# RuntimeRacer/vall-e

Measured on AMD Instinct MI355X. Metric: AR codec-tokens/sec/GPU + NAR 7-stage p50 latency, d=1024 L=12 10s utterance, higher is better.
Workload: dtype bf16

## Files before the change

vall-e_amd/csrc/ar_granules.hpp:

```cpp
#pragma once
#include "ar_kernels.hpp"

namespace vx {

constexpr int FQ_G = 16;
constexpr int FQ_QKV = 192;
constexpr int FQ_PART = 66;
constexpr int FQ_SPIN_MAX = 1 << 18;

typedef unsigned long long fq_gran;

#ifdef VX_STAMPS
}
extern __device__ unsigned long long* g_fq_stamps;
namespace vx {
#endif

__device__ __forceinline__ void gran_store(fq_gran* p, float v, unsigned tag) {
  const fq_gran g = ((fq_gran)tag << 32) | (fq_gran)__float_as_uint(v);
  asm volatile("global_store_dwordx2 %0, %1, off sc1" ::"v"(p), "v"(g) : "memory");
}
__device__ __forceinline__ void gran_load(fq_gran& v, const fq_gran* p) {
  asm volatile("global_load_dwordx2 %0, %1, off sc1" : "=v"(v) : "v"(p) : "memory");
}
// ... 27 lines not shown
```

vall-e_amd/csrc/ar_tp.hpp:

```cpp
#pragma once
#include <type_traits>
#include "ar_granules.hpp"

namespace vx {

#ifdef VX_STAMPS
#define TP_STAMP(which, i)                                                                                            \
  do {                                                                                                                \
    unsigned long long* fq_r_ = g_fq_stamps;                                                                          \
    if (fq_r_ != nullptr && threadIdx.x == 0)                                                                         \
      fq_r_[(((size_t)(which) * 16 + a.layer) * 256 + blockIdx.x) * 16 + (i)] = __builtin_amdgcn_s_memrealtime();      \
  } while (0)
#else
#define TP_STAMP(which, i) do { } while (0)
#endif

constexpr int TP_D = 1024, TP_H = 16, TP_FF = 4096, TP_X = 8, TP_WG = 32;
constexpr int TP_HID = TP_FF / TP_X;
constexpr int TP_ACH = TP_D / TP_X;

struct TpAccArgs {
  long long* add;
  long long* zero;
  const float* bias;
// ... 78 lines not shown
  float s1 = wave_sum_dpp((v.x + v.y) + (v.z + v.w));
  if (lane == 0) red[wave] = s1;
  __syncthreads();
  const float mean = ((red[0] + red[1]) + (red[2] + red[3])) * (1.0f / TP_D);
  const float d0 = v.x - mean, d1 = v.y - mean, d2 = v.z - mean, d3 = v.w - mean;
  float s2 = wave_sum_dpp((d0 * d0 + d1 * d1) + (d2 * d2 + d3 * d3));
  if (lane == 0) red[4 + wave] = s2;
  __syncthreads();
  const float rstd = 1.0f / sqrtf(((red[4] + red[5]) + (red[6] + red[7])) * (1.0f / TP_D) + LN_EPS);
  *reinterpret_cast<float4*>(xs + 4 * tid) =
      make_float4(d0 * rstd * r.g.x + r.be.x, d1 * rstd * r.g.y + r.be.y, d2 * rstd * r.g.z + r.be.z, d3 * rstd * r.g.w + r.be.w);
  __syncthreads();
}

template <bool FIRST>
__device__ __forceinline__ void tp_acc_tail(const TpAccArgs& a, float partial, int xcd, int i, int tid, unsigned long long carry_ll,
                                            float carry_f, float bo) {
  if ((tid & 7) == 0) {
    long long add = tp_fix(partial);
    if (xcd == 0) add += tp_fix(bo) + (FIRST ? tp_fix(carry_f) : (long long)carry_ll);
    atomicAdd(reinterpret_cast<unsigned long long*>(a.add) + 32 * i + (tid >> 3), (unsigned long long)add);
  }
  if (blockIdx.x == 1) {
    *reinterpret_cast<uint4*>(a.zero + 4 * tid) = make_uint4(0u, 0u, 0u, 0u);
    *reinterpret_cast<uint4*>(a.zero + 4 * tid + 2) = make_uint4(0u, 0u, 0u, 0u);
  }
}

template <int KCH, int VEC>
__device__ __forceinline__ void tp_row_read(const float* xs, int lane, float (&xr)[KCH][VEC]) {
#pragma unroll
  for (int c = 0; c < KCH; ++c)
#pragma unroll
    for (int i = 0; i < VEC; i += 4) {
      const float4 t = *reinterpret_cast<const float4*>(xs + (c * 64 + lane) * VEC + i);
      xr[c][i] = t.x; xr[c][i + 1] = t.y; xr[c][i + 2] = t.z; xr[c][i + 3] = t.w;
// ... 1 lines not shown
}
template <typename WT, int KCH>
__device__ __forceinline__ float tp_dot(const uint4 (&w)[KCH], const float (&xr)[KCH][Vec16<WT>::N]) {
  constexpr int VEC = Vec16<WT>::N;
  float s = 0.f;
#pragma unroll
  for (int c = 0; c < KCH; ++c) {
    float wf[VEC];
    unpack<WT>(w[c], wf);
#pragma unroll
    for (int i = 0; i < VEC; ++i) s = fmaf(wf[i], xr[c][i], s);
  }
  return s;
}

template <typename WT, bool FIRST>
__global__ __launch_bounds__(256) void tp_attn_kernel(const void* __restrict__ Wqkv_, const float* __restrict__ x_f32,
                                                      const long long* __restrict__ racc, const float* __restrict__ gbb,
                                                      const ArState* __restrict__ st, const unsigned* __restrict__ epoch,
                                                      const void* __restrict__ Wo_, const TpAttnArgs a) {
  constexpr int VEC = Vec16<WT>::N;
  constexpr int KCH = TP_D / (64 * VEC);
  constexpr int HD = 64;
  constexpr int LPK = HD / VEC, KPW = 64 / LPK, KPB = 4 * KPW, UNR = 4;
  constexpr int NGRP = 4 * KPW;
  constexpr int OCH = TP_ACH / (8 * VEC);
  __shared__ __attribute__((aligned(16))) float xs[TP_D];
  __shared__ float red[8];
  __shared__ __attribute__((aligned(16))) float s_qkv[FQ_QKV];
  __shared__ __attribute__((aligned(16))) float sm_o[NGRP][HD + 4];
  __shared__ float sm_m[4], sm_l[4];
  __shared__ float s_wo[4][HD];
  __shared__ float s_part[2 * FQ_G * FQ_PART];
  __shared__ float s_fac[2 * FQ_G];
  __shared__ __attribute__((aligned(16))) float s_att[TP_ACH];
  const int tid = threadIdx.x, lane = tid & 63, wave = tid >> 6;
  const int x = blockIdx.x & (TP_X - 1), i = blockIdx.x >> 3;
  const int hl = i >> 4, j = i & 15, h = 2 * x + hl;
  const int cih = 4 * j + wave, ch = h * HD + cih;
  const int st_row = st->row, st_done = st->done;
  const unsigned tag = *epoch;
  const WT* __restrict__ W = reinterpret_cast<const WT*>(Wqkv_);

  TpRowLoads rl;
  tp_row_issue<FIRST>(rl, x_f32, racc, gbb, tid);
  TP_STAMP(0, 0);
  vx_u32x4 w[3][KCH];
#pragma unroll
  for (int r = 0; r < 3; ++r)
#pragma unroll
    for (int c = 0; c < KCH; ++c) tp_ld16w(w[r][c], W + (size_t)(r * TP_D + ch) * TP_D + (c * 64 + lane) * VEC);
  float e_bias;
  {
    const float* bp = a.qkv_bias;
    asm volatile("" : "+s"(bp));
    tp_ld4f(e_bias, bp + min(lane, 2) * TP_D + ch);
  }
  unsigned long long carry_ll = 0ull;
  float carry_f = 0.f, bo;
  if (FIRST) tp_ld4f(carry_f, x_f32 + 32 * i + (tid >> 3));
  else asm volatile("global_load_dwordx2 %0, %1, off" : "=v"(carry_ll) : "v"(racc + 32 * i + (tid >> 3)) : "memory");
  tp_ld4f(bo, a.acc.bias + 32 * i + (tid >> 3));
  const int n_old = st_row;
  const int chunk = (n_old + FQ_G - 1) / FQ_G;
  const int j0 = j * chunk, j1 = min(n_old, j0 + chunk);
  const int sub = lane % LPK, grp = lane / LPK;
  vx_u32x4 wo[OCH];
  vx_u32x4 kr[UNR], vr[UNR];
  const WT* kb;
  const WT* vb;
  auto tp_stage2 = [&]() {
    const uint4* wb = reinterpret_cast<const uint4*>(Wo_) + (size_t)(x * TP_WG + i) * OCH * 256;
#pragma unroll
    for (int m = 0; m < OCH; ++m) tp_ld16w(wo[m], wb + m * 256 + tid);
    const void* kcp = a.kcache;
    const void* vcp = a.vcache;
    int ctxm = a.ctx_max;
    asm volatile("" : "+s"(kcp), "+s"(vcp), "+s"(ctxm));
    kb = reinterpret_cast<const WT*>(kcp) + (size_t)h * ctxm * HD + sub * VEC;
    vb = reinterpret_cast<const WT*>(vcp) + (size_t)h * ctxm * HD + sub * VEC;
#pragma unroll
    for (int u = 0; u < UNR; ++u) {
      const int jk = min(j0 + u * KPB + wave * KPW + grp, max(j1, 1) - 1);
      tp_ld16(kr[u], kb + (size_t)jk * HD);
      tp_ld16(vr[u], vb + (size_t)jk * HD);
    }
  };
  tp_stage2();
  auto load_pass = [&](int base) {
#pragma unroll
    for (int u = 0; u < UNR; ++u) {
      const int jk = min(base + u * KPB + wave * KPW + grp, max(j1, 1) - 1);
      const uint4 k4 = ld16(kb + (size_t)jk * HD), v4 = ld16(vb + (size_t)jk * HD);
      kr[u] = vx_u32x4{k4.x, k4.y, k4.z, k4.w};
      vr[u] = vx_u32x4{v4.x, v4.y, v4.z, v4.w};
    }
  };
  constexpr int N_KV = 2 * UNR, N_WO = OCH, N_W = 3 * KCH;

  tp_row_wait<FIRST, N_W + 3 + N_WO + N_KV>(rl);
  TP_STAMP(0, 7);
  tp_row_norm<FIRST>(rl, xs, red, tid);
  TP_STAMP(0, 1);
  {
    float xr[KCH][VEC];
    tp_row_read<KCH, VEC>(xs, lane, xr);
    float acc[3];
#pragma unroll
    for (int r = 0; r < 3; ++r) {
      uint4 wr[KCH];
#pragma unroll
      for (int c = 0; c < KCH; ++c) { tp_wait<N_WO + N_KV + 3>(w[r][c]); wr[c] = tp_u4(w[r][c]); }
      acc[r] = wave_sum_dpp(tp_dot<WT, KCH>(wr, xr));
    }
    tp_wait<N_WO + N_KV + 2>(e_bias);
    if (lane < 3) {
      float v = (lane == 0 ? acc[0] : lane == 1 ? acc[1] : acc[2]) + e_bias;
      if (lane > 0) {
        const WT rv = from_f32<WT>(v);
        v = to_f32(rv);
        if (!st_done) {
          WT* cache = reinterpret_cast<WT*>(lane == 1 ? a.kcache : a.vcache);
          cache[((size_t)h * a.ctx_max + st_row) * HD + cih] = rv;
        }
      }
      gran_store(a.gq + (size_t)h * FQ_QKV + lane * HD + cih, v, tag);
    }
  }
  TP_STAMP(0, 2);
  {
    float v1[1];
    gran_gather<1>(a.gq + (size_t)h * FQ_QKV, FQ_QKV, tag, v1, a.err, 1u);
    if (tid < FQ_QKV) s_qkv[tid] = v1[0];
  }
#pragma unroll
  for (int u = 0; u < UNR; ++u) { tp_wait<0>(kr[u]); tp_wait<0>(vr[u]); }
#pragma unroll
  for (int m = 0; m < OCH; ++m) tp_wait<0>(wo[m]);
  asm volatile("" : "+v"(carry_ll), "+v"(carry_f), "+v"(bo));
  TP_STAMP(0, 3);
  __syncthreads();
  TP_STAMP(0, 8);
  float qv[VEC];
#pragma unroll
  for (int c = 0; c < VEC; ++c) qv[c] = s_qkv[sub * VEC + c] * a.scale;

  float M = -INFINITY, L = 0.f, acc[VEC];
#pragma unroll
  for (int c = 0; c < VEC; ++c) acc[c] = 0.f;
  const bool owner = (j == FQ_G - 1) && wave == 0;
  float sn = -INFINITY;
  if (owner) {
    float dot = 0.f;
#pragma unroll
    for (int c = 0; c < VEC; ++c) dot = fmaf(s_qkv[HD + sub * VEC + c], qv[c], dot);
    sn = (LPK == 8) ? group8_sum_dpp(dot) : group16_sum_dpp(dot);
  }
  for (int base = j0; base < j1 || (owner && base == j0); base += UNR * KPB) {
    if (base != j0) load_pass(base);
    const int nr = (j1 - base + KPB - 1) / KPB;
    float sc[UNR], mloc = (base == j0) ? sn : -INFINITY;
#pragma unroll
    for (int u = 0; u < UNR; ++u) {
      sc[u] = -INFINITY;
      if (u < nr) {
        const int jk = base + u * KPB + wave * KPW + grp;
        float kf[VEC];
        unpack<WT>(tp_u4(kr[u]), kf);
        float dot = 0.f;
#pragma unroll
        for (int c = 0; c < VEC; ++c) dot = fmaf(kf[c], qv[c], dot);
        dot = (LPK == 8) ? group8_sum_dpp(dot) : group16_sum_dpp(dot);
        sc[u] = (jk < j1) ? dot : -INFINITY;
        mloc = fmaxf(mloc, sc[u]);
      }
    }
    mloc = wave_max_dpp(mloc);
    if (mloc != -INFINITY) {
      const float Mn = fmaxf(M, mloc);
      const float corr = (M == -INFINITY) ? 0.f : tp_exp<WT>(M - Mn);
      L *= corr;
#pragma unroll
      for (int c = 0; c < VEC; ++c) acc[c] *= corr;
      M = Mn;
#pragma unroll
      for (int u = 0; u < UNR; ++u)
        if (u < nr) {
          float vf[VEC];
          unpack<WT>(tp_u4(vr[u]), vf);
          const float p = tp_exp<WT>(sc[u] - M);
          L += p;
#pragma unroll
          for (int c = 0; c < VEC; ++c) acc[c] = fmaf(p, vf[c], acc[c]);
        }
      if (owner && base == j0 && grp == 0) {
        const float p = tp_exp<WT>(sn - M);
        L += p;
#pragma unroll
        for (int c = 0; c < VEC; ++c) acc[c] = fmaf(p, s_qkv[2 * HD + sub * VEC + c], acc[c]);
      }
    }
  }
  TP_STAMP(0, 9);
  {
#pragma unroll
    for (int c = 0; c < VEC; c += 4)
      *reinterpret_cast<float4*>(&sm_o[wave * KPW + grp][sub * VEC + c]) = make_float4(acc[c], acc[c + 1], acc[c + 2], acc[c + 3]);
    __builtin_amdgcn_fence(__ATOMIC_RELEASE, "wavefront");
    __builtin_amdgcn_wave_barrier();
    float oc = 0.f;
#pragma unroll
    for (int g = 0; g < KPW; ++g) oc += sm_o[wave * KPW + g][lane];
    const float Lw = wave_sum_dpp(sub == 0 ? L : 0.f);
    s_wo[wave][lane] = oc;
    if (lane == 0) { sm_m[wave] = M; sm_l[wave] = Lw; }
  }
  TP_STAMP(0, 10);
  __syncthreads();
  TP_STAMP(0, 11);
  if (tid < FQ_PART) {
    const float Mx = fmaxf(fmaxf(sm_m[0], sm_m[1]), fmaxf(sm_m[2], sm_m[3]));
    float v = 0.f;
    if (tid == HD) {
      v = Mx;
    } else {
#pragma unroll
      for (int wv = 0; wv < 4; ++wv)
        v = fmaf(tid < HD ? s_wo[wv][tid] : sm_l[wv], (sm_m[wv] == -INFINITY) ? 0.f : tp_exp<WT>(sm_m[wv] - Mx), v);
    }
    gran_store(a.gp + ((size_t)h * FQ_G + j) * FQ_PART + tid, v, tag);
  }
  TP_STAMP(0, 4);
  {
    constexpr int NG = (2 * FQ_G * FQ_PART + 255) / 256;
    float pv[NG];
    gran_gather<NG>(a.gp + (size_t)(2 * x) * FQ_G * FQ_PART, 2 * FQ_G * FQ_PART, tag, pv, a.err, 2u);
#pragma unroll
    for (int g = 0; g < NG; ++g)
      if (tid + 256 * g < 2 * FQ_G * FQ_PART) s_part[tid + 256 * g] = pv[g];
  }
  TP_STAMP(0, 5);
  __syncthreads();
  if (tid < 2 * FQ_G) {
    const float* hp = s_part + (tid >> 4) * FQ_G * FQ_PART;
    float Mx = hp[HD];
#pragma unroll
    for (int s = 1; s < FQ_G; ++s) Mx = fmaxf(Mx, hp[s * FQ_PART + HD]);
    const float pm = hp[(tid & 15) * FQ_PART + HD];
    const float es = (pm == -INFINITY) ? 0.f : tp_exp<WT>(pm - Mx);
    const float Ls = group16_sum_dpp(hp[(tid & 15) * FQ_PART + HD + 1] * es);
    s_fac[tid] = es * (1.0f / Ls);
  }
  __syncthreads();
  if (tid < TP_ACH) {
    const float* hp = s_part + (tid >> 6) * FQ_G * FQ_PART + (tid & 63);
    const float* fp = s_fac + (tid >> 6) * FQ_G;
    float o = 0.f;
#pragma unroll
    for (int s = 0; s < FQ_G; ++s) o = fmaf(hp[s * FQ_PART], fp[s], o);
    s_att[tid] = o;
  }
  __syncthreads();
  {
    float s = 0.f;
#pragma unroll
    for (int m = 0; m < OCH; ++m) {
      float wf[VEC];
      unpack<WT>(tp_u4(wo[m]), wf);
      const float* ap = s_att + ((tid & 7) + 8 * m) * VEC;
#pragma unroll
      for (int c = 0; c < VEC; ++c) s = fmaf(wf[c], ap[c], s);
    }
    s = group8_sum_dpp(s);
    tp_acc_tail<FIRST>(a.acc, s, x, i, tid, carry_ll, carry_f, bo);
  }
  TP_STAMP(0, 6);
}

template <typename WT>
__global__ __launch_bounds__(256) void tp_ffn_kernel(const void* __restrict__ W1_, const long long* __restrict__ racc,
                                                     const float* __restrict__ gbb,
                                                     const unsigned* __restrict__ epoch, const void* __restrict__ W2_,
                                                     const TpFfnArgs a) {
  constexpr int VEC = Vec16<WT>::N;
  constexpr int KCH = TP_D / (64 * VEC);
  constexpr int FCH = TP_HID / (8 * VEC);
  __shared__ __attribute__((aligned(16))) float xs[TP_D];
  __shared__ float red[8];
  __shared__ __attribute__((aligned(16))) float hs[TP_HID];
  const int tid = threadIdx.x, lane = tid & 63, wave = tid >> 6;
  const int x = blockIdx.x & (TP_X - 1), i = blockIdx.x >> 3;
// ... 57 lines not shown
  for (int m = 0; m < FCH; ++m) tp_wait<0>(w2[m]);
  asm volatile("" : "+v"(carry_ll), "+v"(bo));
  TP_STAMP(1, 3);
  __syncthreads();
  {
    float s = 0.f;
#pragma unroll
    for (int m = 0; m < FCH; ++m) {
      float wf[VEC];
      unpack<WT>(tp_u4(w2[m]), wf);
      const float* hp = hs + ((tid & 7) + 8 * m) * VEC;
#pragma unroll
      for (int c = 0; c < VEC; ++c) s = fmaf(wf[c], hp[c], s);
    }
    s = group8_sum_dpp(s);
    tp_acc_tail<false>(a.acc, s, x, i, tid, carry_ll, 0.f, bo);
  }
  TP_STAMP(1, 4);
}

template <typename WT>
__global__ __launch_bounds__(256) void tp_head_kernel(const void* __restrict__ W_, const long long* __restrict__ racc,
                                                      const float* __restrict__ gbb,
                                                      const ArState* __restrict__ st, const TpHeadArgs a) {
  constexpr int VEC = Vec16<WT>::N;
  constexpr int KCH = TP_D / (64 * VEC);
  __shared__ __attribute__((aligned(16))) float xs[TP_D];
  __shared__ float red[8];
  const int tid = threadIdx.x, lane = tid & 63, wave = tid >> 6;
  const WT* __restrict__ W = reinterpret_cast<const WT*>(W_);
  const int row0 = (blockIdx.x * 4 + wave) * 4;
// ... 13 lines not shown
#pragma unroll
  for (int r = 0; r < 4; ++r) {
    uint4 wr[KCH];
#pragma unroll
    for (int c = 0; c < KCH; ++c) { tp_wait<0>(w[r][c]); wr[c] = tp_u4(w[r][c]); }
    acc[r] = wave_sum_dpp(tp_dot<WT, KCH>(wr, xr));
  }
  const int row = row0 + lane;
  if (lane < 4 && row < a.N && !st_done) {
    const float v = lane == 0 ? acc[0] : lane == 1 ? acc[1] : lane == 2 ? acc[2] : acc[3];
    a.logits[row] = v;
    if (st_trace) a.logits[LOGITS_CUR + (size_t)st_pass * a.N + row] = v;
  }
}

template <typename WT>
__global__ void tp_repack_kernel(const WT* __restrict__ src, uint4* __restrict__ dst, int K) {
  constexpr int VEC = Vec16<WT>::N;
  const int KX = K / TP_X, NW = KX / (8 * VEC);
  const size_t word = (size_t)blockIdx.x * 256 + threadIdx.x;
  const size_t total = (size_t)TP_D * K / VEC;
  if (word >= total) return;
  const int t = (int)(word & 255);
  const size_t blk = word >> 8;
  const int m = (int)(blk % NW);
  const int wg = (int)(blk / NW);
  const int x = wg / TP_WG, i = wg % TP_WG;
  const int row = 32 * i + (t >> 3), col = KX * x + ((t & 7) + 8 * m) * VEC;
  dst[word] = *reinterpret_cast<const uint4*>(src + (size_t)row * K + col);
}

}
```

vall-e_amd/csrc/batch_kernels.hpp:

```cpp
#pragma once
#include "common.hpp"
#include "ar_kernels.hpp"
#include "mfma_kernels.hpp"
#include "mx_kernels.hpp"

namespace vx {

constexpr int BMAX = 64;
typedef __bf16 bf16x8b_t __attribute__((ext_vector_type(8)));
typedef float f32x4_t __attribute__((ext_vector_type(4)));

enum BgemmEpi { BE_QKV = 0, BE_RELU = 1, BE_PARTIAL = 2, BE_LOGITS = 3, BE_LOGITS_MAP = 4, BE_BIAS = 5 };

struct BgemmArgs {
  const bf16* A;
  const bf16* W;
  const float* bias;
  int N, K, B;
  int kgroups;
  const ArState* st;
  float* q;
  bf16* kv;
  size_t kv_slot_stride, kv_v_offset;
  int d, hd, ctx_max;
// ... 12 lines not shown
  const uint32_t E = (__float_as_uint(amax) >> 23) & 0xffu;
  uint32_t byte = max(E, 8u) - 8u;
  if (amax * __uint_as_float((254u - byte) << 23) > 448.f) ++byte;
  inv = __uint_as_float((254u - byte) << 23);
  return byte;
}
__device__ __forceinline__ float kv8_scale(uint32_t byte) { return __uint_as_float(byte ? byte << 23 : 0x00400000u); }
__device__ __forceinline__ uint32_t kv8_code(float v) { return (uint32_t)__builtin_amdgcn_cvt_pk_fp8_f32(v, 0.f, 0, false) & 0xffu; }
__device__ __forceinline__ void kv8_unpack(const uint4& r, float (&o)[16]) {
  const uint32_t w[4] = {r.x, r.y, r.z, r.w};
#pragma unroll
  for (int k = 0; k < 4; ++k) {
    const auto lo = __builtin_amdgcn_cvt_pk_f32_fp8((int)w[k], false), hi = __builtin_amdgcn_cvt_pk_f32_fp8((int)w[k], true);
    o[4 * k] = lo[0]; o[4 * k + 1] = lo[1]; o[4 * k + 2] = hi[0]; o[4 * k + 3] = hi[1];
  }
}
__device__ __forceinline__ float group4_sum_dpp(float v) {
  v += dpp_f<0xB1>(0.f, v);
  v += dpp_f<0x4E>(0.f, v);
  return v;
}

template <int EPI, int NS, int NH, bool KV8 = false>
__global__ __launch_bounds__(256) void bgemm_kernel(const bf16* __restrict__ A_, const bf16* __restrict__ W_, unsigned nk, int kgroups,
                                                    const BgemmArgs a) {
  __shared__ float red[4][4 * NH][64];
  const int tid = threadIdx.x, lane = tid & 63, wave = tid >> 6;
  const int c = lane & 15, g = lane >> 4;
  const int ntile = blockIdx.x / kgroups, kg = blockIdx.x - ntile * kgroups;
  const int n0 = ntile * 16;
  const int K = (int)(nk & 0xffffu), Nn = (int)(nk >> 16);
  const int kbeg = kg * (K / kgroups) + wave * NS * 32;
  const bf16* wp = W_ + (size_t)min(n0 + c, Nn - 1) * K + kbeg + 8 * g;
  const bf16* ap = A_ + (size_t)c * K + kbeg + 8 * g;
  float bias_v = 0.f;
// ... 383 lines not shown
```

vall-e_amd/csrc/common.hpp:

```cpp
#pragma once
#include <hip/hip_runtime.h>
#include <stdint.h>

#ifdef VX_STAMPS
extern __device__ unsigned long long g_vx_stamps[32];
#define VX_STAMP(i)                                                                                        \
  do {                                                                                                     \
    if (blockIdx.x == 0 && blockIdx.y == 0 && blockIdx.z == 0 && threadIdx.x == 0) g_vx_stamps[i] = wall_clock64(); \
  } while (0)
extern __device__ unsigned long long* g_vx_kstamps;
#define VX_KSTAMP_WG(kid, st_ptr)                                                                                  \
  do {                                                                                                             \
    if ((kid) >= 0 && (kid) < 64 && blockIdx.x == gridDim.x - 1) {                                                 \
      unsigned long long* vx_r_ = g_vx_kstamps;                                                                    \
      if (vx_r_ != nullptr && threadIdx.x == 0)                                                                    \
        vx_r_[(size_t)(((st_ptr)->pass) & 15) * 64 + (kid)] = __builtin_amdgcn_s_memrealtime();                   \
      return;                                                                                                      \
    }                                                                                                              \
  } while (0)
#define VX_KSTAMP_SELF(kid, pass, t0)                                                                              \
  do {                                                                                                             \
    unsigned long long* vx_r_ = g_vx_kstamps;                                                                      \
    if (vx_r_ != nullptr && (kid) >= 0 && (kid) < 64 && threadIdx.x == 0) vx_r_[(size_t)((pass) & 15) * 64 + (kid)] = (t0); \
  } while (0)
// ... 80 lines not shown
  v = fmaxf(v, dpp_f<0x124>(v, v));
  v = fmaxf(v, dpp_f<0x128>(v, v));
  v = fmaxf(v, dpp_f<0x142, 0xA>(v, v));
  v = fmaxf(v, dpp_f<0x143, 0xC>(v, v));
  return lane63(v);
}
__device__ __forceinline__ uint32_t wave_umin_dpp(uint32_t v) {
  v = min(v, (uint32_t)dpp_i<0xB1>((int)v, (int)v));
  v = min(v, (uint32_t)dpp_i<0x4E>((int)v, (int)v));
  v = min(v, (uint32_t)dpp_i<0x124>((int)v, (int)v));
  v = min(v, (uint32_t)dpp_i<0x128>((int)v, (int)v));
  v = min(v, (uint32_t)dpp_i<0x142, 0xA>((int)v, (int)v));
  v = min(v, (uint32_t)dpp_i<0x143, 0xC>((int)v, (int)v));
  return (uint32_t)__builtin_amdgcn_readlane((int)v, 63);
}
__device__ __forceinline__ float group8_sum_dpp(float v) {
  v += dpp_f<0xB1>(0.f, v);
  v += dpp_f<0x4E>(0.f, v);
  v += dpp_f<0x141>(0.f, v);
  return v;
}
__device__ __forceinline__ float group16_sum_dpp(float v) {
  v = group8_sum_dpp(v);
  v += dpp_f<0x140>(0.f, v);
  return v;
}

__device__ __forceinline__ float wave_sum(float v) {
#pragma unroll
  for (int o = 32; o > 0; o >>= 1) v += __shfl_xor(v, o, WAVE);
  return v;
}
__device__ __forceinline__ float wave_max(float v) {
// ... 94 lines not shown
```

vall-e_amd/csrc/engine.hip:

```cpp
#include <hip/hip_runtime.h>

#include <cmath>
#include <cstdarg>
#include <cstdio>
#include <array>
#include <cstring>
#include <string>
#include <type_traits>
#include <unordered_map>
#include <vector>

#include "host.hpp"
#ifdef VX_STAMPS
__device__ unsigned long long g_vx_stamps[32];
__device__ unsigned long long* g_vx_kstamps = nullptr;
__device__ unsigned long long* g_fq_stamps = nullptr;
#endif
#include "ar_kernels.hpp"
#include "ar_tp.hpp"
#include "rows_kernels.hpp"
#include "mfma_kernels.hpp"
#include "batch_kernels.hpp"
#include "mx_kernels.hpp"
#include "logprob.hpp"
// ... 619 lines not shown
  return VX_OK;
}

extern "C" int vx_finalize_weights(vx_engine* e) {
  if (!e) return fail(VX_ERR_ARG, "null engine");
  ON_DEVICE(e->cfg.device);
  for (auto& k : e->keys)
    if (!e->w[k].set) return fail(VX_ERR_WEIGHTS, "missing key '%s' (strict load)", k.c_str());
  const vx_config& c = e->cfg;
  fill_layers(e, "ar_decoder", c.num_layers, false, e->ar_l);
  if (e->tp) {
    for (int li = 0; li < c.num_layers; ++li) {
      const LayerW& l = e->ar_l[li];
      const unsigned g1 = (unsigned)((size_t)TP_D * TP_D * e->esz / 16 / 256), g2 = (unsigned)((size_t)TP_D * TP_FF * e->esz / 16 / 256);
      if (e->bf16) {
        tp_repack_kernel<bf16><<<g1, 256, 0, e->es>>>((const bf16*)l.out_w, (uint4*)e->tp_wo[li], TP_D);
        tp_repack_kernel<bf16><<<g2, 256, 0, e->es>>>((const bf16*)l.w2, (uint4*)e->tp_w2[li], TP_FF);
      } else {
        tp_repack_kernel<float><<<g1, 256, 0, e->es>>>((const float*)l.out_w, (uint4*)e->tp_wo[li], TP_D);
        tp_repack_kernel<float><<<g2, 256, 0, e->es>>>((const float*)l.w2, (uint4*)e->tp_w2[li], TP_FF);
      }
    }
    auto site = [&](int idx, const float* g, const float* b, const float* bias) -> int {
      float* dst = e->tp_gbb + (size_t)idx * 3 * TP_D;
      HIPC(hipMemcpyAsync(dst, g, TP_D * 4, hipMemcpyDeviceToDevice, e->es));
      HIPC(hipMemcpyAsync(dst + TP_D, b, TP_D * 4, hipMemcpyDeviceToDevice, e->es));
      if (bias) HIPC(hipMemcpyAsync(dst + 2 * TP_D, bias, TP_D * 4, hipMemcpyDeviceToDevice, e->es));
      return VX_OK;
    };
    for (int li = 0; li < c.num_layers; ++li) {
      const LayerW& l = e->ar_l[li];
      VXC(site(2 * li, l.n1_g, l.n1_b, li ? e->ar_l[li - 1].b2 : nullptr));
      VXC(site(2 * li + 1, l.n2_g, l.n2_b, l.out_b));
    }
    VXC(site(2 * c.num_layers, W<float>(e, "ar_decoder.norm.weight"), W<float>(e, "ar_decoder.norm.bias"), e->ar_l.back().b2));
// ... 100 lines not shown
  if ((tv && atoi(tv) == 0) || e->vallf || d != TP_D || H != TP_H || (c.flags & (VX_FLAG_POST_NORM | VX_FLAG_PRENET))) return VX_OK;
  int n1 = 0, n2 = 0;
  if (e->bf16) {
    HIPC(hipOccupancyMaxActiveBlocksPerMultiprocessor(&n1, (const void*)tp_attn_kernel<bf16, true>, 256, 0));
    HIPC(hipOccupancyMaxActiveBlocksPerMultiprocessor(&n2, (const void*)tp_ffn_kernel<bf16>, 256, 0));
  } else {
    HIPC(hipOccupancyMaxActiveBlocksPerMultiprocessor(&n1, (const void*)tp_attn_kernel<float, true>, 256, 0));
    HIPC(hipOccupancyMaxActiveBlocksPerMultiprocessor(&n2, (const void*)tp_ffn_kernel<float>, 256, 0));
  }
  if ((long long)(n1 < n2 ? n1 : n2) * e->num_cu < TP_X * TP_WG) return VX_OK;
  const size_t L = (size_t)c.num_layers;
  VXC(dalloc_t(e, &e->tp_xacc, (size_t)3 * TP_D));
  VXC(dalloc_t(e, &e->tp_gh, L * TP_X * TP_HID));
  VXC(dalloc_t(e, &e->tp_gbb, (2 * L + 1) * 3 * TP_D));
  VXC(dalloc_t(e, &e->fq_gq, L * H * FQ_QKV));
  VXC(dalloc_t(e, &e->fq_gp, L * H * FQ_G * FQ_PART));
  HIPC(hipMemset(e->tp_gbb, 0, (2 * L + 1) * 3 * TP_D * 4));
  HIPC(hipMemset(e->tp_xacc, 0, (size_t)3 * TP_D * sizeof(long long)));
  HIPC(hipMemset(e->tp_gh, 0, L * TP_X * TP_HID * sizeof(fq_gran)));
  HIPC(hipMemset(e->fq_gq, 0, L * H * FQ_QKV * sizeof(fq_gran)));
  HIPC(hipMemset(e->fq_gp, 0, L * H * FQ_G * FQ_PART * sizeof(fq_gran)));
  e->tp_wo.assign(L, nullptr); e->tp_w2.assign(L, nullptr);
  for (size_t li = 0; li < L; ++li) {
    VXC(dalloc(e, &e->tp_wo[li], (size_t)TP_D * TP_D * e->esz));
    VXC(dalloc(e, &e->tp_w2[li], (size_t)TP_D * TP_FF * e->esz));
  }
  e->tp = true;
  return VX_OK;
}

template <typename T>
static int gemm_rows_t(bool mfma, const T* A, const T* Wt, const float* bias, void* C, int M, int N, int K, int epi,
                       bool out_f32, hipStream_t s, void* vt = nullptr, int vt_n0 = 0, int vt_ld = 0) {
  if constexpr (std::is_same<T, bf16>::value) {
    if (mfma) return mfma_gemm_dispatch(A, Wt, bias, C, M, N, K, epi, out_f32, s, (bf16*)vt, vt_n0, vt_ld);
  }
// ... 565 lines not shown
}

static int enqueue_ar_step_tp(vx_engine* e, hipStream_t s) {
  const vx_config& c = e->cfg;
  const int H = c.nhead, hd = c.d_model / H, L = c.num_layers;
  const size_t kv_layer = (size_t)2 * H * e->ctx_max * hd * e->esz;
  const int grid = TP_X * TP_WG;
  auto acc = [&](int n) { return e->tp_xacc + (size_t)(n % 3) * TP_D; };
  for (int li = 0; li < L; ++li) {
    const LayerW& l = e->ar_l[li];
    char* kc = (char*)e->kv + (size_t)li * kv_layer;
    const int n = 2 * li;
    TpAttnArgs a{};
    const float* gbb = e->tp_gbb + (size_t)(2 * li) * 3 * TP_D;
    a.qkv_bias = l.in_b; a.err = e->d_epoch + 1;
    a.gq = e->fq_gq + (size_t)li * H * FQ_QKV; a.gp = e->fq_gp + (size_t)li * H * FQ_G * FQ_PART;
    a.acc.add = acc(n + 1); a.acc.zero = acc(n + 2); a.acc.bias = l.out_b;
    a.kcache = kc; a.vcache = kc + kv_layer / 2; a.ctx_max = e->ctx_max;
    a.scale = 1.0f / sqrtf((float)hd); a.layer = li;
    if (e->bf16) {
      if (li) tp_attn_kernel<bf16, false><<<grid, 256, 0, s>>>(l.in_w, e->ar_x, acc(n), gbb, e->d_st, e->d_epoch, e->tp_wo[li], a);
      else tp_attn_kernel<bf16, true><<<grid, 256, 0, s>>>(l.in_w, e->ar_x, acc(n), gbb, e->d_st, e->d_epoch, e->tp_wo[li], a);
    } else {
      if (li) tp_attn_kernel<float, false><<<grid, 256, 0, s>>>(l.in_w, e->ar_x, acc(n), gbb, e->d_st, e->d_epoch, e->tp_wo[li], a);
      else tp_attn_kernel<float, true><<<grid, 256, 0, s>>>(l.in_w, e->ar_x, acc(n), gbb, e->d_st, e->d_epoch, e->tp_wo[li], a);
    }
    TpFfnArgs f{};
    f.b1 = l.b1; f.err = e->d_epoch + 1; f.gh = e->tp_gh + (size_t)li * TP_X * TP_HID; f.layer = li;
    f.acc.add = acc(n + 2); f.acc.zero = acc(n + 3); f.acc.bias = l.b2;
    if (e->bf16) tp_ffn_kernel<bf16><<<grid, 256, 0, s>>>(l.w1, acc(n + 1), gbb + 3 * TP_D, e->d_epoch, e->tp_w2[li], f);
    else tp_ffn_kernel<float><<<grid, 256, 0, s>>>(l.w1, acc(n + 1), gbb + 3 * TP_D, e->d_epoch, e->tp_w2[li], f);
// ... 1310 lines not shown
  }
  else if (n == "ar_sampled") { src = (const char*)e->d_sampled; size = (int64_t)e->n_pass * 4; }
  else if (n == "ar_argmax") { src = (const char*)e->d_argmax; size = (int64_t)e->n_pass * 4; }
  else if (n == "nar_logits") { src = (const char*)e->nar_logits; size = (int64_t)e->last_T * 1024 * 4; }
  else if (n == "ar_x") { src = (const char*)e->ar_x; size = (int64_t)e->cfg.d_model * 4; }
  else if (n == "nar_x") { src = (const char*)e->X; size = (int64_t)e->last_N * e->cfg.nar_d_model * 4; }
  else if (n == "batch_trace" && e->btrace) { src = (const char*)e->btrace; size = (int64_t)e->bmax * e->btok_stride * AR_VOCAB * 4; }
  else if (n == "batch_logits" && e->bmax > 1) { src = (const char*)e->blogits; size = (int64_t)BMAX * LOGITS_CUR * 4; }
  else if (n == "batch_argmax" && e->bmax > 1) { src = (const char*)e->bargm; size = (int64_t)BMAX * e->btok_stride * 4; }
  else if (n == "batch_sampled" && e->bmax > 1) { src = (const char*)e->bsamp; size = (int64_t)BMAX * e->btok_stride * 4; }
  else if (n == "batch_kv" && e->bmax > 1) {
    src = e->kv8 ? (const char*)e->bkv8 : (const char*)e->bkv;
    size = (int64_t)e->bmax * e->bkv_slot * (e->kv8 ? 1 : 2);
  }
  else if (n == "ar_kv") { src = (const char*)e->kv; size = config_buffer_bytes(e->cfg, n); }
  else if (n == "score_ar_argmax" && e->sc_argmax) { src = (const char*)e->sc_argmax; size = (int64_t)e->sc_rows * 4; }
  else if (n == "batch_kv_scale" && e->kv8) { src = (const char*)e->bkv8s; size = (int64_t)e->bmax * e->bkv_slot / 16; }
  else return fail(VX_ERR_ARG, "unknown buffer '%s'", name);
  if (off < 0 || nbytes < 0 || off + nbytes > size) return fail(VX_ERR_ARG, "read of '%s' out of range (%lld+%lld > %lld)", name, (long long)off, (long long)nbytes, (long long)size);
  HIPC(hipStreamSynchronize(e->es));
  HIPC(hipMemcpy(dst, src + off, (size_t)nbytes, hipMemcpyDeviceToHost));
  return VX_OK;
}

extern "C" int vx_op_convert_bf16(const float* src, void* dst, int64_t n, void* stream) {
  convert_kernel<bf16><<<1024, 256, 0, (hipStream_t)stream>>>(src, (bf16*)dst, (size_t)n);
  HIPC(hipGetLastError());
  return VX_OK;
}

// ... 951 lines not shown
```

Measured before the change: 4528.

## Split attention over 8 KV slices per head and repack Wo per head

Attention for each head is now spread over 8 sequence slices instead of 16. Only half the workgroups per head run flash-decoding, and the rest skip the KV work and go straight to the out-projection. The out-projection weights are repacked so each workgroup reduces a single head's 64-wide attention output over 64 output rows, rather than gathering both heads' partials. This cuts the size of the cross-workgroup granule gather and the dependency on the other head. The cost is twice as much KV traversal per active workgroup, so attention across long contexts has less parallelism.

```diff
diff --git a/vall-e_amd/csrc/ar_granules.hpp b/vall-e_amd/csrc/ar_granules.hpp
--- a/vall-e_amd/csrc/ar_granules.hpp
+++ b/vall-e_amd/csrc/ar_granules.hpp
@@ -4,6 +4,7 @@
 namespace vx {
 
 constexpr int FQ_G = 16;
+constexpr int FQ_S = 8;
 constexpr int FQ_QKV = 192;
 constexpr int FQ_PART = 66;
 constexpr int FQ_SPIN_MAX = 1 << 18;
diff --git a/vall-e_amd/csrc/ar_tp.hpp b/vall-e_amd/csrc/ar_tp.hpp
--- a/vall-e_amd/csrc/ar_tp.hpp
+++ b/vall-e_amd/csrc/ar_tp.hpp
@@ -116,12 +116,12 @@
 }
 
 template <bool FIRST>
-__device__ __forceinline__ void tp_acc_tail(const TpAccArgs& a, float partial, int xcd, int i, int tid, unsigned long long carry_ll,
-                                            float carry_f, float bo) {
-  if ((tid & 7) == 0) {
+__device__ __forceinline__ void tp_acc_tail(const TpAccArgs& a, float partial, bool writer, int row, bool lead, int tid,
+                                            unsigned long long carry_ll, float carry_f, float bo) {
+  if (writer) {
     long long add = tp_fix(partial);
-    if (xcd == 0) add += tp_fix(bo) + (FIRST ? tp_fix(carry_f) : (long long)carry_ll);
-    atomicAdd(reinterpret_cast<unsigned long long*>(a.add) + 32 * i + (tid >> 3), (unsigned long long)add);
+    if (lead) add += tp_fix(bo) + (FIRST ? tp_fix(carry_f) : (long long)carry_ll);
+    atomicAdd(reinterpret_cast<unsigned long long*>(a.add) + row, (unsigned long long)add);
   }
   if (blockIdx.x == 1) {
     *reinterpret_cast<uint4*>(a.zero + 4 * tid) = make_uint4(0u, 0u, 0u, 0u);
@@ -153,26 +153,31 @@
   return s;
 }
 
-template <typename WT, bool FIRST>
-__global__ __launch_bounds__(256) void tp_attn_kernel(const void* __restrict__ Wqkv_, const float* __restrict__ x_f32,
-                                                      const long long* __restrict__ racc, const float* __restrict__ gbb,
-                                                      const ArState* __restrict__ st, const unsigned* __restrict__ epoch,
-                                                      const void* __restrict__ Wo_, const TpAttnArgs a) {
+template <int NGRP> struct TpAttnSmem {
+  __attribute__((aligned(16))) float xs[TP_D];
+  float red[8];
+  __attribute__((aligned(16))) float s_qkv[FQ_QKV];
+  __attribute__((aligned(16))) float sm_o[NGRP][64 + 4];
+  float sm_m[4], sm_l[4];
+  float s_wo[4][64];
+  float s_part[FQ_S * FQ_PART];
+  float s_fac[FQ_S];
+  __attribute__((aligned(16))) float s_att[64];
+};
+
+template <typename WT, bool FIRST, bool ATT>
+__device__ __forceinline__ void tp_attn_body(const void* __restrict__ Wqkv_, const float* __restrict__ x_f32,
+                                             const long long* __restrict__ racc, const float* __restrict__ gbb,
+                                             const ArState* __restrict__ st, const unsigned* __restrict__ epoch,
+                                             const void* __restrict__ Wo_, const TpAttnArgs& a,
+                                             TpAttnSmem<4 * Vec16<WT>::N>& sm) {
   constexpr int VEC = Vec16<WT>::N;
   constexpr int KCH = TP_D / (64 * VEC);
   constexpr int HD = 64;
   constexpr int LPK = HD / VEC, KPW = 64 / LPK, KPB = 4 * KPW, UNR = 4;
-  constexpr int NGRP = 4 * KPW;
-  constexpr int OCH = TP_ACH / (8 * VEC);
-  __shared__ __attribute__((aligned(16))) float xs[TP_D];
-  __shared__ float red[8];
-  __shared__ __attribute__((aligned(16))) float s_qkv[FQ_QKV];
-  __shared__ __attribute__((aligned(16))) float sm_o[NGRP][HD + 4];
-  __shared__ float sm_m[4], sm_l[4];
-  __shared__ float s_wo[4][HD];
-  __shared__ float s_part[2 * FQ_G * FQ_PART];
-  __shared__ float s_fac[2 * FQ_G];
-  __shared__ __attribute__((aligned(16))) float s_att[TP_ACH];
+  constexpr int OCH = HD / (4 * VEC);
+  float* const xs = sm.xs;
+  float* const s_qkv = sm.s_qkv;
   const int tid = threadIdx.x, lane = tid & 63, wave = tid >> 6;
   const int x = blockIdx.x & (TP_X - 1), i = blockIdx.x >> 3;
   const int hl = i >> 4, j = i & 15, h = 2 * x + hl;
@@ -195,23 +200,26 @@
     asm volatile("" : "+s"(bp));
     tp_ld4f(e_bias, bp + min(lane, 2) * TP_D + ch);
   }
+  const int orow = 64 * j + (tid >> 2);
   unsigned long long carry_ll = 0ull;
   float carry_f = 0.f, bo;
-  if (FIRST) tp_ld4f(carry_f, x_f32 + 32 * i + (tid >> 3));
-  else asm volatile("global_load_dwordx2 %0, %1, off" : "=v"(carry_ll) : "v"(racc + 32 * i + (tid >> 3)) : "memory");
-  tp_ld4f(bo, a.acc.bias + 32 * i + (tid >> 3));
+  if (FIRST) tp_ld4f(carry_f, x_f32 + orow);
+  else asm volatile("global_load_dwordx2 %0, %1, off" : "=v"(carry_ll) : "v"(racc + orow) : "memory");
+  tp_ld4f(bo, a.acc.bias + orow);
   const int n_old = st_row;
-  const int chunk = (n_old + FQ_G - 1) / FQ_G;
+  const int chunk = (n_old + FQ_S - 1) / FQ_S;
   const int j0 = j * chunk, j1 = min(n_old, j0 + chunk);
   const int sub = lane % LPK, grp = lane / LPK;
   vx_u32x4 wo[OCH];
   vx_u32x4 kr[UNR], vr[UNR];
   const WT* kb;
   const WT* vb;
-  auto tp_stage2 = [&]() {
+  {
     const uint4* wb = reinterpret_cast<const uint4*>(Wo_) + (size_t)(x * TP_WG + i) * OCH * 256;
 #pragma unroll
     for (int m = 0; m < OCH; ++m) tp_ld16w(wo[m], wb + m * 256 + tid);
+  }
+  if constexpr (ATT) {
     const void* kcp = a.kcache;
     const void* vcp = a.vcache;
     int ctxm = a.ctx_max;
@@ -224,8 +232,7 @@
       tp_ld16(kr[u], kb + (size_t)jk * HD);
       tp_ld16(vr[u], vb + (size_t)jk * HD);
     }
-  };
-  tp_stage2();
+  }
   auto load_pass = [&](int base) {
 #pragma unroll
     for (int u = 0; u < UNR; ++u) {
@@ -235,11 +242,11 @@
       vr[u] = vx_u32x4{v4.x, v4.y, v4.z, v4.w};
     }
   };
-  constexpr int N_KV = 2 * UNR, N_WO = OCH, N_W = 3 * KCH;
+  constexpr int N_KV = ATT ? 2 * UNR : 0, N_WO = OCH, N_W = 3 * KCH;
 
   tp_row_wait<FIRST, N_W + 3 + N_WO + N_KV>(rl);
   TP_STAMP(0, 7);
-  tp_row_norm<FIRST>(rl, xs, red, tid);
+  tp_row_norm<FIRST>(rl, xs, sm.red, tid);
   TP_STAMP(0, 1);
   {
     float xr[KCH][VEC];
@@ -267,137 +274,144 @@
     }
   }
   TP_STAMP(0, 2);
-  {
-    float v1[1];
-    gran_gather<1>(a.gq + (size_t)h * FQ_QKV, FQ_QKV, tag, v1, a.err, 1u);
-    if (tid < FQ_QKV) s_qkv[tid] = v1[0];
-  }
-#pragma unroll
-  for (int u = 0; u < UNR; ++u) { tp_wait<0>(kr[u]); tp_wait<0>(vr[u]); }
-#pragma unroll
-  for (int m = 0; m < OCH; ++m) tp_wait<0>(wo[m]);
-  asm volatile("" : "+v"(carry_ll), "+v"(carry_f), "+v"(bo));
-  TP_STAMP(0, 3);
-  __syncthreads();
-  TP_STAMP(0, 8);
-  float qv[VEC];
-#pragma unroll
-  for (int c = 0; c < VEC; ++c) qv[c] = s_qkv[sub * VEC + c] * a.scale;
-
-  float M = -INFINITY, L = 0.f, acc[VEC];
-#pragma unroll
-  for (int c = 0; c < VEC; ++c) acc[c] = 0.f;
-  const bool owner = (j == FQ_G - 1) && wave == 0;
-  float sn = -INFINITY;
-  if (owner) {
-    float dot = 0.f;
-#pragma unroll
-    for (int c = 0; c < VEC; ++c) dot = fmaf(s_qkv[HD + sub * VEC + c], qv[c], dot);
-    sn = (LPK == 8) ? group8_sum_dpp(dot) : group16_sum_dpp(dot);
-  }
-  for (int base = j0; base < j1 || (owner && base == j0); base += UNR * KPB) {
-    if (base != j0) load_pass(base);
-    const int nr = (j1 - base + KPB - 1) / KPB;
-    float sc[UNR], mloc = (base == j0) ? sn : -INFINITY;
-#pragma unroll
-    for (int u = 0; u < UNR; ++u) {
-      sc[u] = -INFINITY;
-      if (u < nr) {
-        const int jk = base + u * KPB + wave * KPW + grp;
-        float kf[VEC];
-        unpack<WT>(tp_u4(kr[u]), kf);
-        float dot = 0.f;
-#pragma unroll
-        for (int c = 0; c < VEC; ++c) dot = fmaf(kf[c], qv[c], dot);
-        dot = (LPK == 8) ? group8_sum_dpp(dot) : group16_sum_dpp(dot);
-        sc[u] = (jk < j1) ? dot : -INFINITY;
-        mloc = fmaxf(mloc, sc[u]);
+  if constexpr (ATT) {
+    {
+      float v1[1];
+      gran_gather<1>(a.gq + (size_t)h * FQ_QKV, FQ_QKV, tag, v1, a.err, 1u);
+      if (tid < FQ_QKV) s_qkv[tid] = v1[0];
+    }
+#pragma unroll
+    for (int u = 0; u < UNR; ++u) { tp_wait<0>(kr[u]); tp_wait<0>(vr[u]); }
+#pragma unroll
+    for (int m = 0; m < OCH; ++m) tp_wait<0>(wo[m]);
+    asm volatile("" : "+v"(carry_ll), "+v"(carry_f), "+v"(bo));
+    TP_STAMP(0, 3);
+    __syncthreads();
+    TP_STAMP(0, 8);
+    float qv[VEC];
+#pragma unroll
+    for (int c = 0; c < VEC; ++c) qv[c] = s_qkv[sub * VEC + c] * a.scale;
+
+    float M = -INFINITY, L = 0.f, acc[VEC];
+#pragma unroll
+    for (int c = 0; c < VEC; ++c) acc[c] = 0.f;
+    const bool owner = (j == FQ_S - 1) && wave == 0;
+    float sn = -INFINITY;
+    if (owner) {
+      float dot = 0.f;
+#pragma unroll
+      for (int c = 0; c < VEC; ++c) dot = fmaf(s_qkv[HD + sub * VEC + c], qv[c], dot);
+      sn = (LPK == 8) ? group8_sum_dpp(dot) : group16_sum_dpp(dot);
+    }
+    for (int base = j0; base < j1 || (owner && base == j0); base += UNR * KPB) {
+      if (base != j0) load_pass(base);
+      const int nr = (j1 - base + KPB - 1) / KPB;
+      float sc[UNR], mloc = (base == j0) ? sn : -INFINITY;
+#pragma unroll
+      for (int u = 0; u < UNR; ++u) {
+        sc[u] = -INFINITY;
+        if (u < nr) {
+          const int jk = base + u * KPB + wave * KPW + grp;
+          float kf[VEC];
+          unpack<WT>(tp_u4(kr[u]), kf);
+          float dot = 0.f;
+#pragma unroll
+          for (int c = 0; c < VEC; ++c) dot = fmaf(kf[c], qv[c], dot);
+          dot = (LPK == 8) ? group8_sum_dpp(dot) : group16_sum_dpp(dot);
+          sc[u] = (jk < j1) ? dot : -INFINITY;
+          mloc = fmaxf(mloc, sc[u]);
+        }
       }
-    }
-    mloc = wave_max_dpp(mloc);
-    if (mloc != -INFINITY) {
-      const float Mn = fmaxf(M, mloc);
-      const float corr = (M == -INFINITY) ? 0.f : tp_exp<WT>(M - Mn);
-      L *= corr;
-#pragma unroll
-      for (int c = 0; c < VEC; ++c) acc[c] *= corr;
-      M = Mn;
-#pragma unroll
-      for (int u = 0; u < UNR; ++u)
-        if (u < nr) {
-          float vf[VEC];
-          unpack<WT>(tp_u4(vr[u]), vf);
-          const float p = tp_exp<WT>(sc[u] - M);
+      mloc = wave_max_dpp(mloc);
+      if (mloc != -INFINITY) {
+        const float Mn = fmaxf(M, mloc);
+        const float corr = (M == -INFINITY) ? 0.f : tp_exp<WT>(M - Mn);
+        L *= corr;
+#pragma unroll
+        for (int c = 0; c < VEC; ++c) acc[c] *= corr;
+        M = Mn;
+#pragma unroll
+        for (int u = 0; u < UNR; ++u)
+          if (u < nr) {
+            float vf[VEC];
+            unpack<WT>(tp_u4(vr[u]), vf);
+            const float p = tp_exp<WT>(sc[u] - M);
+            L += p;
+#pragma unroll
+            for (int c = 0; c < VEC; ++c) acc[c] = fmaf(p, vf[c], acc[c]);
+          }
+        if (owner && base == j0 && grp == 0) {
+          const float p = tp_exp<WT>(sn - M);
           L += p;
 #pragma unroll
-          for (int c = 0; c < VEC; ++c) acc[c] = fmaf(p, vf[c], acc[c]);
+          for (int c = 0; c < VEC; ++c) acc[c] = fmaf(p, s_qkv[2 * HD + sub * VEC + c], acc[c]);
         }
-      if (owner && base == j0 && grp == 0) {
-        const float p = tp_exp<WT>(sn - M);
-        L += p;
-#pragma unroll
-        for (int c = 0; c < VEC; ++c) acc[c] = fmaf(p, s_qkv[2 * HD + sub * VEC + c], acc[c]);
       }
     }
-  }
-  TP_STAMP(0, 9);
-  {
-#pragma unroll
-    for (int c = 0; c < VEC; c += 4)
-      *reinterpret_cast<float4*>(&sm_o[wave * KPW + grp][sub * VEC + c]) = make_float4(acc[c], acc[c + 1], acc[c + 2], acc[c + 3]);
-    __builtin_amdgcn_fence(__ATOMIC_RELEASE, "wavefront");
-    __builtin_amdgcn_wave_barrier();
-    float oc = 0.f;
-#pragma unroll
-    for (int g = 0; g < KPW; ++g) oc += sm_o[wave * KPW + g][lane];
-    const float Lw = wave_sum_dpp(sub == 0 ? L : 0.f);
-    s_wo[wave][lane] = oc;
-    if (lane == 0) { sm_m[wave] = M; sm_l[wave] = Lw; }
-  }
-  TP_STAMP(0, 10);
-  __syncthreads();
-  TP_STAMP(0, 11);
-  if (tid < FQ_PART) {
-    const float Mx = fmaxf(fmaxf(sm_m[0], sm_m[1]), fmaxf(sm_m[2], sm_m[3]));
-    float v = 0.f;
-    if (tid == HD) {
-      v = Mx;
-    } else {
-#pragma unroll
-      for (int wv = 0; wv < 4; ++wv)
-        v = fmaf(tid < HD ? s_wo[wv][tid] : sm_l[wv], (sm_m[wv] == -INFINITY) ? 0.f : tp_exp<WT>(sm_m[wv] - Mx), v);
-    }
-    gran_store(a.gp + ((size_t)h * FQ_G + j) * FQ_PART + tid, v, tag);
-  }
-  TP_STAMP(0, 4);
-  {
-    constexpr int NG = (2 * FQ_G * FQ_PART + 255) / 256;
+    TP_STAMP(0, 9);
+    {
+#pragma unroll
+      for (int c = 0; c < VEC; c += 4)
+        *reinterpret_cast<float4*>(&sm.sm_o[wave * KPW + grp][sub * VEC + c]) = make_float4(acc[c], acc[c + 1], acc[c + 2], acc[c + 3]);
+      __builtin_amdgcn_fence(__ATOMIC_RELEASE, "wavefront");
+      __builtin_amdgcn_wave_barrier();
+      float oc = 0.f;
+#pragma unroll
+      for (int g = 0; g < KPW; ++g) oc += sm.sm_o[wave * KPW + g][lane];
+      const float Lw = wave_sum_dpp(sub == 0 ? L : 0.f);
+      sm.s_wo[wave][lane] = oc;
+      if (lane == 0) { sm.sm_m[wave] = M; sm.sm_l[wave] = Lw; }
+    }
+    TP_STAMP(0, 10);
+    __syncthreads();
+    TP_STAMP(0, 11);
+    if (tid < FQ_PART) {
+      const float Mx = fmaxf(fmaxf(sm.sm_m[0], sm.sm_m[1]), fmaxf(sm.sm_m[2], sm.sm_m[3]));
+      float v = 0.f;
+      if (tid == HD) {
+        v = Mx;
+      } else {
+#pragma unroll
+        for (int wv = 0; wv < 4; ++wv)
+          v = fmaf(tid < HD ? sm.s_wo[wv][tid] : sm.sm_l[wv], (sm.sm_m[wv] == -INFINITY) ? 0.f : tp_exp<WT>(sm.sm_m[wv] - Mx), v);
+      }
+      gran_store(a.gp + ((size_t)h * FQ_S + j) * FQ_PART + tid, v, tag);
+    }
+    TP_STAMP(0, 4);
+  } else {
+    TP_STAMP(0, 3); TP_STAMP(0, 8); TP_STAMP(0, 9); TP_STAMP(0, 10); TP_STAMP(0, 11); TP_STAMP(0, 4);
+  }
+  {
+    constexpr int NG = (FQ_S * FQ_PART + 255) / 256;
     float pv[NG];
-    gran_gather<NG>(a.gp + (size_t)(2 * x) * FQ_G * FQ_PART, 2 * FQ_G * FQ_PART, tag, pv, a.err, 2u);
+    gran_gather<NG>(a.gp + (size_t)h * FQ_S * FQ_PART, FQ_S * FQ_PART, tag, pv, a.err, 2u);
 #pragma unroll
     for (int g = 0; g < NG; ++g)
-      if (tid + 256 * g < 2 * FQ_G * FQ_PART) s_part[tid + 256 * g] = pv[g];
+      if (tid + 256 * g < FQ_S * FQ_PART) sm.s_part[tid + 256 * g] = pv[g];
+  }
+  if constexpr (!ATT) {
+#pragma unroll
+    for (int m = 0; m < OCH; ++m) tp_wait<0>(wo[m]);
+    asm volatile("" : "+v"(carry_ll), "+v"(carry_f), "+v"(bo));
   }
   TP_STAMP(0, 5);
   __syncthreads();
-  if (tid < 2 * FQ_G) {
-    const float* hp = s_part + (tid >> 4) * FQ_G * FQ_PART;
+  if (tid < FQ_S) {
+    const float* hp = sm.s_part;
     float Mx = hp[HD];
 #pragma unroll
-    for (int s = 1; s < FQ_G; ++s) Mx = fmaxf(Mx, hp[s * FQ_PART + HD]);
-    const float pm = hp[(tid & 15) * FQ_PART + HD];
+    for (int s = 1; s < FQ_S; ++s) Mx = fmaxf(Mx, hp[s * FQ_PART + HD]);
+    const float pm = hp[tid * FQ_PART + HD];
     const float es = (pm == -INFINITY) ? 0.f : tp_exp<WT>(pm - Mx);
-    const float Ls = group16_sum_dpp(hp[(tid & 15) * FQ_PART + HD + 1] * es);
-    s_fac[tid] = es * (1.0f / Ls);
-  }
-  __syncthreads();
-  if (tid < TP_ACH) {
-    const float* hp = s_part + (tid >> 6) * FQ_G * FQ_PART + (tid & 63);
-    const float* fp = s_fac + (tid >> 6) * FQ_G;
+    const float Ls = group8_sum_dpp(hp[tid * FQ_PART + HD + 1] * es);
+    sm.s_fac[tid] = es * (1.0f / Ls);
+  }
+  __syncthreads();
+  if (tid < HD) {
     float o = 0.f;
 #pragma unroll
-    for (int s = 0; s < FQ_G; ++s) o = fmaf(hp[s * FQ_PART], fp[s], o);
-    s_att[tid] = o;
+    for (int s = 0; s < FQ_S; ++s) o = fmaf(sm.s_part[s * FQ_PART + tid], sm.s_fac[s], o);
+    sm.s_att[tid] = o;
   }
   __syncthreads();
   {
@@ -406,14 +420,24 @@
     for (int m = 0; m < OCH; ++m) {
       float wf[VEC];
       unpack<WT>(tp_u4(wo[m]), wf);
-      const float* ap = s_att + ((tid & 7) + 8 * m) * VEC;
+      const float* ap = sm.s_att + ((tid & 3) + 4 * m) * VEC;
 #pragma unroll
       for (int c = 0; c < VEC; ++c) s = fmaf(wf[c], ap[c], s);
     }
-    s = group8_sum_dpp(s);
-    tp_acc_tail<FIRST>(a.acc, s, x, i, tid, carry_ll, carry_f, bo);
+    s = group4_sum_dpp(s);
+    tp_acc_tail<FIRST>(a.acc, s, (tid & 3) == 0, orow, h == 0, tid, carry_ll, carry_f, bo);
   }
   TP_STAMP(0, 6);
+}
+
+template <typename WT, bool FIRST>
+__global__ __launch_bounds__(256) void tp_attn_kernel(const void* __restrict__ Wqkv_, const float* __restrict__ x_f32,
+                                                      const long long* __restrict__ racc, const float* __restrict__ gbb,
+                                                      const ArState* __restrict__ st, const unsigned* __restrict__ epoch,
+                                                      const void* __restrict__ Wo_, const TpAttnArgs a) {
+  __shared__ TpAttnSmem<4 * Vec16<WT>::N> sm;
+  if (((blockIdx.x >> 3) & (FQ_G - 1)) < FQ_S) tp_attn_body<WT, FIRST, true>(Wqkv_, x_f32, racc, gbb, st, epoch, Wo_, a, sm);
+  else tp_attn_body<WT, FIRST, false>(Wqkv_, x_f32, racc, gbb, st, epoch, Wo_, a, sm);
 }
 
 template <typename WT>
@@ -501,7 +525,7 @@
       for (int c = 0; c < VEC; ++c) s = fmaf(wf[c], hp[c], s);
     }
     s = group8_sum_dpp(s);
-    tp_acc_tail<false>(a.acc, s, x, i, tid, carry_ll, 0.f, bo);
+    tp_acc_tail<false>(a.acc, s, (tid & 7) == 0, 32 * i + (tid >> 3), x == 0, tid, carry_ll, 0.f, bo);
   }
   TP_STAMP(1, 4);
 }
@@ -545,7 +569,7 @@
   }
 }
 
-template <typename WT>
+template <typename WT, bool HEADS>
 __global__ void tp_repack_kernel(const WT* __restrict__ src, uint4* __restrict__ dst, int K) {
   constexpr int VEC = Vec16<WT>::N;
   const int KX = K / TP_X, NW = KX / (8 * VEC);
@@ -557,7 +581,14 @@
   const int m = (int)(blk % NW);
   const int wg = (int)(blk / NW);
   const int x = wg / TP_WG, i = wg % TP_WG;
-  const int row = 32 * i + (t >> 3), col = KX * x + ((t & 7) + 8 * m) * VEC;
+  int row, col;
+  if (HEADS) {
+    row = 64 * (i & 15) + (t >> 2);
+    col = 64 * (2 * x + (i >> 4)) + ((t & 3) + 4 * m) * VEC;
+  } else {
+    row = 32 * i + (t >> 3);
+    col = KX * x + ((t & 7) + 8 * m) * VEC;
+  }
   dst[word] = *reinterpret_cast<const uint4*>(src + (size_t)row * K + col);
 }
 
diff --git a/vall-e_amd/csrc/batch_kernels.hpp b/vall-e_amd/csrc/batch_kernels.hpp
--- a/vall-e_amd/csrc/batch_kernels.hpp
+++ b/vall-e_amd/csrc/batch_kernels.hpp
@@ -50,11 +50,6 @@
     const auto lo = __builtin_amdgcn_cvt_pk_f32_fp8((int)w[k], false), hi = __builtin_amdgcn_cvt_pk_f32_fp8((int)w[k], true);
     o[4 * k] = lo[0]; o[4 * k + 1] = lo[1]; o[4 * k + 2] = hi[0]; o[4 * k + 3] = hi[1];
   }
-}
-__device__ __forceinline__ float group4_sum_dpp(float v) {
-  v += dpp_f<0xB1>(0.f, v);
-  v += dpp_f<0x4E>(0.f, v);
-  return v;
 }
 
 template <int EPI, int NS, int NH, bool KV8 = false>
diff --git a/vall-e_amd/csrc/common.hpp b/vall-e_amd/csrc/common.hpp
--- a/vall-e_amd/csrc/common.hpp
+++ b/vall-e_amd/csrc/common.hpp
@@ -118,9 +118,13 @@
   v = min(v, (uint32_t)dpp_i<0x143, 0xC>((int)v, (int)v));
   return (uint32_t)__builtin_amdgcn_readlane((int)v, 63);
 }
-__device__ __forceinline__ float group8_sum_dpp(float v) {
+__device__ __forceinline__ float group4_sum_dpp(float v) {
   v += dpp_f<0xB1>(0.f, v);
   v += dpp_f<0x4E>(0.f, v);
+  return v;
+}
+__device__ __forceinline__ float group8_sum_dpp(float v) {
+  v = group4_sum_dpp(v);
   v += dpp_f<0x141>(0.f, v);
   return v;
 }
diff --git a/vall-e_amd/csrc/engine.hip b/vall-e_amd/csrc/engine.hip
--- a/vall-e_amd/csrc/engine.hip
+++ b/vall-e_amd/csrc/engine.hip
@@ -657,11 +657,11 @@
       const LayerW& l = e->ar_l[li];
       const unsigned g1 = (unsigned)((size_t)TP_D * TP_D * e->esz / 16 / 256), g2 = (unsigned)((size_t)TP_D * TP_FF * e->esz / 16 / 256);
       if (e->bf16) {
-        tp_repack_kernel<bf16><<<g1, 256, 0, e->es>>>((const bf16*)l.out_w, (uint4*)e->tp_wo[li], TP_D);
-        tp_repack_kernel<bf16><<<g2, 256, 0, e->es>>>((const bf16*)l.w2, (uint4*)e->tp_w2[li], TP_FF);
+        tp_repack_kernel<bf16, true><<<g1, 256, 0, e->es>>>((const bf16*)l.out_w, (uint4*)e->tp_wo[li], TP_D);
+        tp_repack_kernel<bf16, false><<<g2, 256, 0, e->es>>>((const bf16*)l.w2, (uint4*)e->tp_w2[li], TP_FF);
       } else {
-        tp_repack_kernel<float><<<g1, 256, 0, e->es>>>((const float*)l.out_w, (uint4*)e->tp_wo[li], TP_D);
-        tp_repack_kernel<float><<<g2, 256, 0, e->es>>>((const float*)l.w2, (uint4*)e->tp_w2[li], TP_FF);
+        tp_repack_kernel<float, true><<<g1, 256, 0, e->es>>>((const float*)l.out_w, (uint4*)e->tp_wo[li], TP_D);
+        tp_repack_kernel<float, false><<<g2, 256, 0, e->es>>>((const float*)l.w2, (uint4*)e->tp_w2[li], TP_FF);
       }
     }
     auto site = [&](int idx, const float* g, const float* b, const float* bias) -> int {
@@ -792,12 +792,12 @@
   VXC(dalloc_t(e, &e->tp_gh, L * TP_X * TP_HID));
   VXC(dalloc_t(e, &e->tp_gbb, (2 * L + 1) * 3 * TP_D));
   VXC(dalloc_t(e, &e->fq_gq, L * H * FQ_QKV));
-  VXC(dalloc_t(e, &e->fq_gp, L * H * FQ_G * FQ_PART));
+  VXC(dalloc_t(e, &e->fq_gp, L * H * FQ_S * FQ_PART));
   HIPC(hipMemset(e->tp_gbb, 0, (2 * L + 1) * 3 * TP_D * 4));
   HIPC(hipMemset(e->tp_xacc, 0, (size_t)3 * TP_D * sizeof(long long)));
   HIPC(hipMemset(e->tp_gh, 0, L * TP_X * TP_HID * sizeof(fq_gran)));
   HIPC(hipMemset(e->fq_gq, 0, L * H * FQ_QKV * sizeof(fq_gran)));
-  HIPC(hipMemset(e->fq_gp, 0, L * H * FQ_G * FQ_PART * sizeof(fq_gran)));
+  HIPC(hipMemset(e->fq_gp, 0, L * H * FQ_S * FQ_PART * sizeof(fq_gran)));
   e->tp_wo.assign(L, nullptr); e->tp_w2.assign(L, nullptr);
   for (size_t li = 0; li < L; ++li) {
     VXC(dalloc(e, &e->tp_wo[li], (size_t)TP_D * TP_D * e->esz));
@@ -1393,7 +1393,7 @@
     TpAttnArgs a{};
     const float* gbb = e->tp_gbb + (size_t)(2 * li) * 3 * TP_D;
     a.qkv_bias = l.in_b; a.err = e->d_epoch + 1;
-    a.gq = e->fq_gq + (size_t)li * H * FQ_QKV; a.gp = e->fq_gp + (size_t)li * H * FQ_G * FQ_PART;
+    a.gq = e->fq_gq + (size_t)li * H * FQ_QKV; a.gp = e->fq_gp + (size_t)li * H * FQ_S * FQ_PART;
     a.acc.add = acc(n + 1); a.acc.zero = acc(n + 2); a.acc.bias = l.out_b;
     a.kcache = kc; a.vcache = kc + kv_layer / 2; a.ctx_max = e->ctx_max;
     a.scale = 1.0f / sqrtf((float)hd); a.layer = li;
@@ -2734,6 +2734,7 @@
     size = (int64_t)e->bmax * e->bkv_slot * (e->kv8 ? 1 : 2);
   }
   else if (n == "ar_kv") { src = (const char*)e->kv; size = config_buffer_bytes(e->cfg, n); }
+  else if (n == "tp_wo" && e->tp) { src = (const char*)e->tp_wo[0]; size = (int64_t)TP_D * TP_D * e->esz; }
   else if (n == "score_ar_argmax" && e->sc_argmax) { src = (const char*)e->sc_argmax; size = (int64_t)e->sc_rows * 4; }
   else if (n == "batch_kv_scale" && e->kv8) { src = (const char*)e->bkv8s; size = (int64_t)e->bmax * e->bkv_slot / 16; }
   else return fail(VX_ERR_ARG, "unknown buffer '%s'", name);
```

Result: faster. 4873, median of 6 (+7.6%).
